# ShuangXieIrene/ssds.pytorch

Hardware: AMD Instinct MI355X
Metric: images/sec (fwd+decode+NMS) SSD-MobileNetV2@512 (higher is better)
Workload: dtype bf16

## Files before the change

ssds.pytorch_amd/csrc/ssdk_flow_common.h:

```cpp
#pragma once
#include "ssdk_common.h"

namespace ssdk {

typedef __bf16 fl_bf16x8 __attribute__((ext_vector_type(8)));
typedef _Float16 fl_f16x8 __attribute__((ext_vector_type(8)));
typedef float f32x4 __attribute__((ext_vector_type(4)));
typedef _Float16 fl_h2 __attribute__((ext_vector_type(2)));

struct FlowParams {
  const u16* x;
  u16* y;
  const u16* we;
  const float* se;
  const float* be;
  const u16* wd;
  const u16* bd;
  const u16* wp;
  const float* sp;
  const float* bp;
  int N, H, W, Cin, Chid, Cout, Ho, Wo, residual;
  int strips, segs, rs;
  int Himg, Wimg, Cimg, layout;
  unsigned long long seg_mask;
// ... 13 lines not shown
  if constexpr (DT == SSDK_BF16) {
    u32 b = __builtin_bit_cast(u32, v);
    if ((b & 0x7fffffffu) > 0x7f800000u) return (b >> 16) | 0x40u;
    return (b + 0x7fffu + ((b >> 16) & 1u)) >> 16;
  } else {
    _Float16 h = (_Float16)v;
    return (u32)__builtin_bit_cast(u16, h);
  }
}
typedef float fl_f32x2 __attribute__((ext_vector_type(2)));
typedef __bf16 fl_bf16x2 __attribute__((ext_vector_type(2)));
template <int DT> __device__ __forceinline__ u32 fl_pack2(float a, float b) {
  const fl_f32x2 v = {a, b};
  if constexpr (DT == SSDK_BF16) return __builtin_bit_cast(u32, __builtin_convertvector(v, fl_bf16x2));
  else return __builtin_bit_cast(u32, __builtin_convertvector(v, fl_h2));
}
template <int DT> __device__ __forceinline__ float fl_from16(u32 h) {
  if constexpr (DT == SSDK_BF16) return bf16_bits_to_f32(h);
  else return f16_bits_to_f32(h);
}
__device__ __forceinline__ u32 fl_from_left(u32 v) { return (u32)__builtin_amdgcn_update_dpp(0, (int)v, 0x111, 0xf, 0xf, true); }
__device__ __forceinline__ u32 fl_from_right(u32 v) { return (u32)__builtin_amdgcn_update_dpp(0, (int)v, 0x101, 0xf, 0xf, true); }

typedef float fl_f2 __attribute__((ext_vector_type(2)));
constexpr float kFlSixth = 1.0f / 6.0f;
__device__ __forceinline__ u32 fl_unit_pack(float a, float b, fl_f2 k) {
  const fl_f2 v = {a, b};
  fl_f2 r;
  asm("v_pk_mul_f32 %0, %1, %2 clamp" : "=v"(r) : "v"(v), "v"(k));
  return __builtin_bit_cast(u32, __builtin_amdgcn_cvt_pkrtz(r[0], r[1]));
}
__device__ __forceinline__ fl_h2 fl_fma_clamp01(fl_h2 a, fl_h2 b, fl_h2 c) {
  fl_h2 r;
  asm("v_pk_fma_f16 %0, %1, %2, %3 clamp" : "=v"(r) : "v"(a), "v"(b), "v"(c));
  return r;
}
__device__ __forceinline__ u32 fl_sixth_h2(u32 w) {
  return fl_to16<SSDK_F16>(fl_from16<SSDK_F16>(w & 0xffffu) * kFlSixth) | (fl_to16<SSDK_F16>(fl_from16<SSDK_F16>(w >> 16) * kFlSixth) << 16);
}

}
```

ssds.pytorch_amd/csrc/ssdk_mbflow.hip:

```cpp
#include <stdio.h>
#include <atomic>
#include <type_traits>

#include "ssdk_common.h"
#include "ssdk_flow_common.h"

namespace ssdk {

constexpr int kFlowThreads = 256;

template <int NCH, int NFO>
struct FlowLds {
  static constexpr int T = (NCH + 1) / 2;
  static constexpr int we = 0;
  static constexpr int sb = we + NCH * 1024;
  static constexpr int wd = sb + NCH * 4 * 32;
  static constexpr int bd = wd + NCH * 9 * 4 * 8;
  static constexpr int wp = (bd + NCH * 4 * 8 + 15) & ~15;
  static constexpr int spb = wp + NFO * T * 1024;
  static constexpr int bytes = spb + NFO * 4 * 32;
};

template <int DT, int S, int NCH, int NFO, int NS, bool STEM = false, bool YE = false, bool PAIR = false, bool XD = false>
__global__ __launch_bounds__(kFlowThreads, ((STEM && !YE) || PAIR) ? 3 : 2) void mbflow_kernel(const FlowParams p) {
  static_assert(!PAIR || (S == 1 && !STEM), "row pairs: stride-1 blocks");
  static_assert(!XD || (STEM && !YE), "dword image loads: the stem's interior instance");
  using L = FlowLds<NCH, NFO>;
  constexpr int T = L::T;
  extern __shared__ __attribute__((aligned(16))) unsigned char smem[];
  const u32 tid = threadIdx.x, lane = tid & 63u, wave = tid >> 6;
  const u32 fr = lane & 15u, fg = lane >> 4;
  const int Cin = p.Cin, Chid = p.Chid, Cout = p.Cout;

  for (u32 i = tid; i < (u32)(NCH * 64); i += kFlowThreads) {
    const u32 c = i >> 6, l = i & 63u, hc = c * 16 + (l & 15u), k0 = (l >> 4) * 8;
    u32x4 v = {0u, 0u, 0u, 0u};
    if constexpr (STEM) {
      if (hc < (u32)Chid) {
#pragma unroll
        for (u32 j = 0; j < 8; ++j) {
          u32 ci, ky, kx;
          bool kv;
          if constexpr (XD) {
            const u32 g = k0 >> 3;
            u32 t;
            if (j < 3u) {
              t = 2u * g;
              kx = j == 2u ? 0u : j + 1u;
// ... 72 lines not shown
    }
    *reinterpret_cast<f32x4*>(smem + L::spb + i * 32) = s;
    *reinterpret_cast<f32x4*>(smem + L::spb + i * 32 + 16) = b;
  }
  __syncthreads();

  const u32 item = blockIdx.x * (kFlowThreads / 64) + (u32)__builtin_amdgcn_readfirstlane((int)wave);
  const int groups = (p.strips + NS - 1) / NS;
  const int nseg = STEM ? __builtin_popcountll(p.seg_mask) : p.segs;
  const u32 per_img = (u32)(groups * nseg);
  if (item >= (u32)p.N * per_img) return;
  const int n = (int)(item / per_img), rem = (int)(item % per_img);
  int seg = rem / groups;
  const int grp = rem % groups;
  if constexpr (STEM) {
    unsigned long long m = p.seg_mask;
    for (int i = 0; i < seg; ++i) m &= m - 1;
    seg = __builtin_ctzll(m);
  }
  constexpr int OW = S == 1 ? 14 : 7;
  constexpr bool MERGE = S == 2 && NS == 2;
  constexpr int NA = MERGE ? 1 : NS;
  const int oy0 = seg * p.rs, oy1 = (oy0 + p.rs < p.Ho ? oy0 + p.rs : p.Ho) - 1;
  int ix[NS], oxl[NA];
  bool col_ok[NS], out_lane[NA];
#pragma unroll
  for (int s = 0; s < NS; ++s) {
    const int strip = grp * NS + s;
    const int ox0 = strip * OW;
    ix[s] = MERGE ? 2 * (grp * 15 + (int)fr) - s : ox0 * S - 1 + (int)fr;
    col_ok[s] = strip < p.strips && (unsigned)ix[s] < (unsigned)p.W;
    if constexpr (!MERGE) {
      oxl[s] = S == 1 ? ox0 + (int)fr - 1 : ox0 + ((int)fr - 1) / 2;
      out_lane[s] = strip < p.strips && (S == 1 ? (fr >= 1u && fr <= 14u) : ((fr & 1u) && fr <= 13u)) && oxl[s] < p.Wo;
    }
  }
  if constexpr (MERGE) {
    oxl[0] = grp * 15 + (int)fr;
    out_lane[0] = fr <= 14u && oxl[0] < p.Wo;
  }

  const u16* ximg = STEM ? p.x + (size_t)n * p.Cimg * p.Himg * p.Wimg : p.x + (size_t)n * p.H * p.W * Cin;
  const bool k_ok = fg * 8u < (u32)Cin;
  constexpr u32 kOOR = 0x40000000u;
  u32 xoff[STEM ? NS : 1][STEM ? 8 : 1], xoff0[(STEM && !YE) ? NS : 1][(STEM && !YE) ? 8 : 1], kyM[STEM ? 3 : 1];
  const int pstr = STEM ? (p.layout == 1 ? 1 : p.Cimg) : 0, cstr = STEM ? (p.layout == 1 ? p.Himg * p.Wimg : 1) : 0;
  if constexpr (STEM) {
    kyM[0] = kyM[1] = kyM[2] = 0u;
#pragma unroll
    for (int j = 0; j < 8; ++j) {
      const u32 k = fg * 8u + (u32)j, ci = k / 9u, ky = (k % 9u) / 3u, kx = k % 3u;
      const bool kv = k < 27u && ci < (u32)p.Cimg;
      const u32 vo = (u32)(2 * (int)fr * pstr + (int)ci * cstr + ((int)ky * p.Wimg + (int)kx) * pstr) * 2u;
      kyM[0] |= (kv && ky == 0u) ? (1u << j) : 0u;
      kyM[1] |= (kv && ky == 1u) ? (1u << j) : 0u;
      kyM[2] |= (kv && ky == 2u) ? (1u << j) : 0u;
#pragma unroll
      for (int s = 0; s < NS; ++s) {
        xoff[s][j] = (kv && col_ok[s] && (unsigned)(2 * ix[s] - 1 + (int)kx) < (unsigned)p.Wimg) ? vo : kOOR;
        if constexpr (!YE) xoff0[s][j] = ky == 0u ? kOOR : xoff[s][j];
      }
    }
  }
  u32 xd_off[XD ? NS : 1][3], xd_off0[XD ? NS : 1][2], xd_edge[2], xd_edge0[2];
  if constexpr (XD) {
    const u32 tA = 2u * fg, tB = 2u * fg + 1u;
    auto voff = [&](u32 t, int shift, int s_) -> u32 {
      const u32 ci = t / 3u, ky = t % 3u;
      const int px = ix[s_] - shift;
      const bool ok = ci < (u32)p.Cimg && grp * NS + s_ < p.strips && (unsigned)px < (unsigned)p.W;
      return ok ? (u32)((2 * (int)fr + (int)ci * p.Himg * p.Wimg + (int)ky * p.Wimg) * 2 + 4 * (1 - shift)) : kOOR;
    };
#pragma unroll
    for (int s = 0; s < NS; ++s) {
      xd_off[s][0] = voff(tA, 0, s);
      xd_off[s][1] = voff(tB, 0, s);
      xd_off[s][2] = fg == 0u ? voff(8u, 0, s) : (fg == 1u ? voff(8u, 1, s) : kOOR);
      xd_off0[s][0] = tA % 3u == 0u ? kOOR : xd_off[s][0];
      xd_off0[s][1] = tB % 3u == 0u ? kOOR : xd_off[s][1];
    }
    xd_edge[0] = fr == 0u ? voff(tA, 1, 0) : kOOR;
    xd_edge[1] = fr == 0u ? voff(tB, 1, 0) : kOOR;
    xd_edge0[0] = tA % 3u == 0u ? kOOR : xd_edge[0];
    xd_edge0[1] = tB % 3u == 0u ? kOOR : xd_edge[1];
  }
  const int xmargin = STEM ? (p.Wimg + 8) * pstr * 2 : 0;
  const __amdgpu_buffer_rsrc_t xrsrc = __builtin_amdgcn_make_buffer_rsrc(
      (void*)(reinterpret_cast<const unsigned char*>(ximg) - xmargin), 0, STEM ? p.Cimg * p.Himg * p.Wimg * 2 + xmargin : 0, 0x00020000);
  constexpr int XW = STEM ? 8 : 4;
  struct XRow {
    u32 w[XW];
  };
  auto load_x = [&](int iy, int s) -> XRow {
    XRow out;
#pragma unroll
    for (int q = 0; q < XW; ++q) out.w[q] = 0u;
    if constexpr (STEM) {
      const int strip = grp * NS + s;
      const int base = ((2 * iy - 1) * p.Wimg + (2 * (strip * 14 - 1) - 1)) * pstr;
      if constexpr (XD) {
        const bool row_in = (unsigned)iy < (unsigned)p.H, top = iy == 0;
        const int soff = row_in ? (base + 1) * 2 + xmargin - 4 : (int)kOOR;
        out.w[0] = (u32)__builtin_amdgcn_raw_buffer_load_b32(xrsrc, (int)(top ? xd_off0[s][0] : xd_off[s][0]), soff, 0);
        out.w[1] = (u32)__builtin_amdgcn_raw_buffer_load_b32(xrsrc, (int)(top ? xd_off0[s][1] : xd_off[s][1]), soff, 0);
        out.w[2] = (u32)__builtin_amdgcn_raw_buffer_load_b32(xrsrc, (int)xd_off[s][2], soff, 0);
        if (s == 0) {
          out.w[3] = (u32)__builtin_amdgcn_raw_buffer_load_b32(xrsrc, (int)(top ? xd_edge0[0] : xd_edge[0]), soff, 0);
          out.w[4] = (u32)__builtin_amdgcn_raw_buffer_load_b32(xrsrc, (int)(top ? xd_edge0[1] : xd_edge[1]), soff, 0);
        }
        return out;
      } else if constexpr (YE) {
        u32 rowmask = 0;
#pragma unroll
        for (int ky = 0; ky < 3; ++ky)
          rowmask |= ((unsigned)iy < (unsigned)p.H && (unsigned)(2 * iy - 1 + ky) < (unsigned)p.Himg) ? kyM[ky] : 0u;
#pragma unroll
        for (int j = 0; j < 8; ++j) {
          const u32 off = (((rowmask >> j) & 1u) && xoff[s][j] != kOOR) ? xoff[s][j] + (u32)(base * 2 + xmargin) : kOOR;
          out.w[j] = (u32)__builtin_amdgcn_raw_buffer_load_b16(xrsrc, (int)off, 0, 0);
        }
      } else {
        const bool row_in = (unsigned)iy < (unsigned)p.H, top = iy == 0;
        const int soff = row_in ? base * 2 + xmargin : (int)kOOR;
// ... 4 lines not shown
      return out;
    } else {
      if (k_ok && col_ok[s] && (unsigned)iy < (unsigned)p.H) {
        const u32x4 v = *reinterpret_cast<const u32x4*>(ximg + ((size_t)iy * p.W + ix[s]) * Cin + fg * 8);
        out.w[0] = v[0];
        out.w[1] = v[1];
        out.w[2] = v[2];
        out.w[3] = v[3];
      }
      return out;
    }
  };

  const bool dbgw = p.dbg != nullptr && blockIdx.x == gridDim.x / 2 && __builtin_amdgcn_readfirstlane((int)wave) == 0;
  int dbg_k = 0;
  fl_h2 accA[NA][NCH * 2], accB[NA][NCH * 2], accC[NA][NCH * 2];
  fl_h2 accD[PAIR ? NA : 1][PAIR ? NCH * 2 : 1];

  auto row = [&](const XRow (&xraw)[NS], int iy, auto FINc, auto MIDc, auto INIc, fl_h2 (&fin)[NA][NCH * 2],
                 fl_h2 (&mid)[NA][NCH * 2], fl_h2 (&ini)[NA][NCH * 2], int oy_fin) {
    constexpr bool FIN = decltype(FINc)::value, MID = decltype(MIDc)::value, INI = decltype(INIc)::value;
    if (dbgw && dbg_k < 250) {
      p.dbg[dbg_k++] = __builtin_readcyclecounter();
      if constexpr (STEM) asm volatile("s_waitcnt vmcnt(16)" ::: "memory");
      else asm volatile("s_waitcnt vmcnt(2)" ::: "memory");
      p.dbg[dbg_k++] = __builtin_readcyclecounter();
    }
    u32x4 xf[NS];
#pragma unroll
    for (int s = 0; s < NS; ++s) {
      if constexpr (XD) {
        int oa, ob;
        if (s == 0) {
          oa = (int)xraw[0].w[3];
          ob = (int)xraw[0].w[4];
        } else {
          oa = __builtin_amdgcn_update_dpp(0, (int)xraw[s - 1].w[0], 0x123, 0xf, 0xf, true);
          ob = __builtin_amdgcn_update_dpp(0, (int)xraw[s - 1].w[1], 0x123, 0xf, 0xf, true);
        }
        const u32 an = (u32)__builtin_amdgcn_update_dpp(oa, (int)xraw[s].w[0], 0x111, 0xf, 0xf, false);
        const u32 bn = (u32)__builtin_amdgcn_update_dpp(ob, (int)xraw[s].w[1], 0x111, 0xf, 0xf, false);
        xf[s][0] = xraw[s].w[0];
        xf[s][1] = __builtin_amdgcn_perm(bn, an, 0x07060302u);
        xf[s][2] = xraw[s].w[1];
        xf[s][3] = fg == 1u ? (xraw[s].w[2] & 0xffff0000u) : xraw[s].w[2];
      } else if constexpr (STEM) {
#pragma unroll
        for (int q = 0; q < 4; ++q) xf[s][q] = xraw[s].w[2 * q] | (xraw[s].w[2 * q + 1] << 16);
      } else {
#pragma unroll
        for (int q = 0; q < 4; ++q) xf[s][q] = xraw[s].w[q];
      }
    }
    fl_f2 hi[NS];
#pragma unroll
    for (int s = 0; s < NS; ++s) {
      const float k = (col_ok[s] && (unsigned)iy < (unsigned)p.H) ? kFlSixth : 0.f;
      hi[s] = fl_f2{k, k};
    }
    const bool store_row = FIN && oy_fin >= oy0 && oy_fin <= oy1;
    uint2 resv[NA][NFO];
    if (!STEM && !MERGE && FIN && store_row && p.residual) {
#pragma unroll
      for (int s = 0; s < NA; ++s)
#pragma unroll
        for (int f = 0; f < NFO; ++f) {
          const int co = f * 16 + (int)fg * 4;
          uint2 r = make_uint2(0u, 0u);
// ... 38 lines not shown
          fl_h2 s0 = init ? fl_as_h2(bdi.x) : a0, s1 = init ? fl_as_h2(bdi.y) : a1;
          s0 = __builtin_elementwise_fma(l0, fl_as_h2(w0.x), s0);
          s1 = __builtin_elementwise_fma(l1, fl_as_h2(w0.y), s1);
          s0 = __builtin_elementwise_fma(c0, fl_as_h2(w1.x), s0);
          s1 = __builtin_elementwise_fma(c1, fl_as_h2(w1.y), s1);
          if (ky == 2) {
            s0 = fl_fma_clamp01(r0, fl_as_h2(w2.x), s0);
            s1 = fl_fma_clamp01(r1, fl_as_h2(w2.y), s1);
          } else {
            s0 = __builtin_elementwise_fma(r0, fl_as_h2(w2.x), s0);
            s1 = __builtin_elementwise_fma(r1, fl_as_h2(w2.y), s1);
          }
          asm volatile("" : "+v"(s0), "+v"(s1));
          a0 = s0;
          a1 = s1;
        };
        if constexpr (INI) taps(0, ini[a][2 * c], ini[a][2 * c + 1], true);
        if constexpr (MID) taps(1, mid[a][2 * c], mid[a][2 * c + 1], false);
        if constexpr (FIN) taps(2, fin[a][2 * c], fin[a][2 * c + 1], false);
      };
      if constexpr (MERGE) {
        fold(fl_as_h2(ew[1][0]), fl_as_h2(ew[1][1]), fl_as_h2(ew[0][0]), fl_as_h2(ew[0][1]), fl_as_h2(fl_from_right(ew[1][0])),
             fl_as_h2(fl_from_right(ew[1][1])), 0);
      } else {
#pragma unroll
        for (int s = 0; s < NS; ++s)
          fold(fl_as_h2(fl_from_left(ew[s][0])), fl_as_h2(fl_from_left(ew[s][1])), fl_as_h2(ew[s][0]), fl_as_h2(ew[s][1]),
               fl_as_h2(fl_from_right(ew[s][0])), fl_as_h2(fl_from_right(ew[s][1])), s);
      }
#pragma unroll
      for (int s = 0; s < NS; ++s) e_cur[s] = e_nxt[s];
      __builtin_amdgcn_sched_barrier(0);
    }
    if (dbgw && dbg_k < 250) p.dbg[dbg_k++] = __builtin_readcyclecounter();
    if constexpr (FIN) {
      if (store_row) {
        asm volatile("" ::: "memory");
        f32x4 yacc[NA][NFO];
#pragma unroll
        for (int s = 0; s < NA; ++s)
#pragma unroll
          for (int f = 0; f < NFO; ++f) yacc[s][f] = f32x4{0.f, 0.f, 0.f, 0.f};
#pragma unroll
        for (int t = 0; t < T; ++t) {
          u32x4 db[NA];
#pragma unroll
// ... 196 lines not shown
          for (int o = 0; o < 2; ++o)
#pragma unroll
            for (int s = 0; s < NA; ++s) {
              if (!(st[o] && out_lane[s])) continue;
              u16* yrow = p.y + (((size_t)n * p.Ho + (iy - 1 + o)) * p.Wo + oxl[s]) * Cout;
              u32 h01 = fl_pack2<DT>(fmaf(yacc[o][s][f][0], spv[0], bpv[0]), fmaf(yacc[o][s][f][1], spv[1], bpv[1]));
              u32 h23 = fl_pack2<DT>(fmaf(yacc[o][s][f][2], spv[2], bpv[2]), fmaf(yacc[o][s][f][3], spv[3], bpv[3]));
              if (p.residual) {
                const u32 x01 = resv[o][s][f].x, x23 = resv[o][s][f].y;
                h01 = fl_pack2<DT>(fl_from16<DT>(h01 & 0xffffu) + fl_from16<DT>(x01 & 0xffffu), fl_from16<DT>(h01 >> 16) + fl_from16<DT>(x01 >> 16));
                h23 = fl_pack2<DT>(fl_from16<DT>(h23 & 0xffffu) + fl_from16<DT>(x23 & 0xffffu), fl_from16<DT>(h23 >> 16) + fl_from16<DT>(x23 >> 16));
              }
              *reinterpret_cast<uint2*>(yrow + co) = make_uint2(h01, h23);
            }
        }
      }
    }
    if (dbgw && dbg_k < 250) p.dbg[dbg_k++] = __builtin_readcyclecounter();
  };

  const auto Y = std::true_type{};
  const auto No = std::false_type{};
  auto load_row = [&](XRow (&dst)[NS], int iy) {
#pragma unroll
    for (int s = 0; s < NS; ++s) dst[s] = load_x(iy, s);
  };
  XRow xa[NS], xb[NS];
  {
    if constexpr (PAIR) {
      const int rend = oy1 + 1;
      XRow xc[NS], xd[NS];
      load_row(xa, oy0 - 1);
      load_row(xb, oy0);
      for (int r = oy0 - 1; r <= rend; r += 4) {
        load_row(xc, r + 2);
        load_row(xd, r + 3);
        row2(xa, xb, r, accA, accB, accC, accD);
        load_row(xa, r + 4);
        load_row(xb, r + 5);
        row2(xc, xd, r + 2, accC, accD, accA, accB);
      }
    } else if constexpr (S == 1) {
      const int rend = oy1 + 1;
      load_row(xa, oy0 - 1);
      for (int r = oy0 - 1; r <= rend; r += 6) {
        load_row(xb, r + 1);
// ... 8 lines not shown
        row(xa, r + 4, Y, Y, Y, accB, accC, accA, r + 3);
        load_row(xa, r + 6);
        row(xb, r + 5, Y, Y, Y, accC, accA, accB, r + 4);
      }
    } else {
      const int rend = 2 * oy1 + 1;
      load_row(xa, 2 * oy0 - 1);
      for (int r = 2 * oy0 - 1; r <= rend; r += 4) {
        load_row(xb, r + 1);
        row(xa, r, Y, No, Y, accA, accC, accB, (r - 1) / 2);
        load_row(xa, r + 2);
        row(xb, r + 1, No, Y, No, accC, accB, accC, 0);
        load_row(xb, r + 3);
        row(xa, r + 2, Y, No, Y, accB, accC, accA, (r + 1) / 2);
        load_row(xa, r + 4);
        row(xb, r + 3, No, Y, No, accC, accA, accC, 0);
      }
    }
  }
}

constexpr int kFlowNS = 2;

template <int DT, int S, int NCH, int NFO>
static void flow_launch(const FlowParams& p, unsigned grid, hipStream_t stream) {
  constexpr int lds = FlowLds<NCH, NFO>::bytes;
  if constexpr (S == 1 && NCH == 9) {
    if (p.layout == 101) {
      static const int pair = getenv("SSDK_FLOW_PAIR") ? atoi(getenv("SSDK_FLOW_PAIR")) : 1;
      if (pair) {
        (void)hipFuncSetAttribute(reinterpret_cast<const void*>(&mbflow_kernel<DT, S, NCH, NFO, 1, false, false, true>), hipFuncAttributeMaxDynamicSharedMemorySize, lds);
        hipLaunchKernelGGL((mbflow_kernel<DT, S, NCH, NFO, 1, false, false, true>), dim3(grid), dim3(kFlowThreads), lds, stream, p);
        return;
      }
      (void)hipFuncSetAttribute(reinterpret_cast<const void*>(&mbflow_kernel<DT, S, NCH, NFO, 1>), hipFuncAttributeMaxDynamicSharedMemorySize, lds);
      hipLaunchKernelGGL((mbflow_kernel<DT, S, NCH, NFO, 1>), dim3(grid), dim3(kFlowThreads), lds, stream, p);
      return;
    }
  }
  (void)hipFuncSetAttribute(reinterpret_cast<const void*>(&mbflow_kernel<DT, S, NCH, NFO, kFlowNS>), hipFuncAttributeMaxDynamicSharedMemorySize, lds);
  hipLaunchKernelGGL((mbflow_kernel<DT, S, NCH, NFO, kFlowNS>), dim3(grid), dim3(kFlowThreads), lds, stream, p);
}

template <int DT, int S>
static bool flow_dispatch(const FlowParams& p, int nch, int nfo, unsigned grid, hipStream_t stream) {
#define SSDK_FLOW(NCH_, NFO_)                                   \
  if (nch == NCH_ && nfo == NFO_) {                             \
    flow_launch<DT, S, NCH_, NFO_>(p, grid, stream);            \
    return true;                                                \
  }
  SSDK_FLOW(6, 2)
  SSDK_FLOW(9, 2)
  SSDK_FLOW(12, 2)
  SSDK_FLOW(12, 4)
#undef SSDK_FLOW
  return false;
}

int launch_mbflow(const ssdk_mbconv_desc* d, hipStream_t stream) {
// ... 45 lines not shown
    if (!dbg_dev) (void)hipMalloc(&dbg_dev, 256 * sizeof(unsigned long long));
    (void)hipMemsetAsync(dbg_dev, 0, 256 * sizeof(unsigned long long), stream);
    p.dbg = dbg_dev;
  }
  auto dbg_print = [&]() {
    if (!env_dbg) return;
    unsigned long long hh[256];
    (void)hipStreamSynchronize(stream);
    (void)hipMemcpy(hh, dbg_dev, sizeof(hh), hipMemcpyDeviceToHost);
    fprintf(stderr, "[mbflow dbg] Cin=%d Chid=%d Cout=%d s=%d stem=%d rs=%d: per row (wait x | chunks | project+store | to next row):", d->Cin,
            d->Chid, d->Cout, d->stride, (int)stem, p.rs);
    for (int i = 0; i + 4 < 250 && hh[i + 4]; i += 4)
      fprintf(stderr, " [%llu %llu %llu %llu]", hh[i + 1] - hh[i], hh[i + 2] - hh[i + 1], hh[i + 3] - hh[i + 2], hh[i + 4] - hh[i + 3]);
    fprintf(stderr, "\n");
  };
  const int ow = d->stride == 1 ? 14 : 7;
  p.strips = (p.Wo + ow - 1) / ow;
  if (d->stride == 2) p.strips = 2 * ((p.Wo + 14) / 15);
  constexpr int env_rs = 0;
  constexpr int env_ns1 = 1;
  const bool ns1 = ((env_ns1 & 1) && !stem && d->stride == 1 && nch == 9) || ((env_ns1 & 2) && stem);
  const int flow_ns = ns1 ? 1 : kFlowNS;
  if (ns1 && !stem) p.layout = 101;
  const int groups = (p.strips + flow_ns - 1) / flow_ns;
  int rs = 64;
  while (rs > 16 && (long)d->N * groups * ((p.Ho + rs - 1) / rs) < 4096) rs >>= 1;
  if ((long)d->N * groups * ((p.Ho + rs - 1) / rs) < 2048 && env_rs <= 0 && variant <= 0) return 1;
  if (variant > 0) {
    while (rs > 8 && (long)d->N * groups * ((p.Ho + rs - 1) / rs) < 2048) rs >>= 1;
  }
  if (env_rs > 0) rs = env_rs;
  if (rs > p.Ho) rs = p.Ho;
  p.rs = rs;
  p.segs = (p.Ho + rs - 1) / rs;
  const long items = (long)d->N * groups * p.segs;
  const unsigned grid = (unsigned)((items + 3) / 4);
  bool ok;
  if (stem) {
    if (p.segs > 64) return 1;
    unsigned long long edge = 0;
    for (int sgi = 0; sgi < p.segs; ++sgi) {
      const int o0 = sgi * p.rs, o1 = (o0 + p.rs < p.Ho ? o0 + p.rs : p.Ho) - 1;
      const int last_row = o1 + 1 < p.H - 1 ? o1 + 1 : p.H - 1;
      if (2 * last_row + 1 >= p.Himg) edge |= 1ull << sgi;
    }
    const unsigned long long all = p.segs == 64 ? ~0ull : ((1ull << p.segs) - 1ull);
    constexpr int lds = FlowLds<2, 1>::bytes;
    auto go = [&](auto DTc, auto YEc, unsigned long long mask) {
      constexpr int DTv = decltype(DTc)::value;
      constexpr bool YEv = decltype(YEc)::value;
      if (!mask) return;
      FlowParams q = p;
      q.seg_mask = mask;
      const long it = (long)d->N * groups * __builtin_popcountll(mask);
      const unsigned g = (unsigned)((it + 3) / 4);
      if (ns1) {
        (void)hipFuncSetAttribute(reinterpret_cast<const void*>(&mbflow_kernel<DTv, 1, 2, 1, 1, true, YEv>),
                                  hipFuncAttributeMaxDynamicSharedMemorySize, lds);
        hipLaunchKernelGGL((mbflow_kernel<DTv, 1, 2, 1, 1, true, YEv>), dim3(g), dim3(kFlowThreads), lds, stream, q);
        return;
      }
      if constexpr (!YEv) {
        static const int env_xd = getenv("SSDK_STEM_DWORD") ? atoi(getenv("SSDK_STEM_DWORD")) : 1;
        if (env_xd && q.layout == 1 && (q.Wimg & 1) == 0 && (reinterpret_cast<uintptr_t>(q.x) & 3u) == 0) {
          (void)hipFuncSetAttribute(reinterpret_cast<const void*>(&mbflow_kernel<DTv, 1, 2, 1, kFlowNS, true, false, false, true>),
                                    hipFuncAttributeMaxDynamicSharedMemorySize, lds);
          hipLaunchKernelGGL((mbflow_kernel<DTv, 1, 2, 1, kFlowNS, true, false, false, true>), dim3(g), dim3(kFlowThreads), lds, stream, q);
          return;
        }
      }
      (void)hipFuncSetAttribute(reinterpret_cast<const void*>(&mbflow_kernel<DTv, 1, 2, 1, kFlowNS, true, YEv>),
                                hipFuncAttributeMaxDynamicSharedMemorySize, lds);
      hipLaunchKernelGGL((mbflow_kernel<DTv, 1, 2, 1, kFlowNS, true, YEv>), dim3(g), dim3(kFlowThreads), lds, stream, q);
    };
    if (d->dtype == SSDK_BF16) {
      go(std::integral_constant<int, SSDK_BF16>{}, std::false_type{}, all & ~edge);
      go(std::integral_constant<int, SSDK_BF16>{}, std::true_type{}, edge);
    } else {
      go(std::integral_constant<int, SSDK_F16>{}, std::false_type{}, all & ~edge);
      go(std::integral_constant<int, SSDK_F16>{}, std::true_type{}, edge);
    }
    dbg_print();
    return 0;
  }
  if (d->dtype == SSDK_BF16) ok = d->stride == 1 ? flow_dispatch<SSDK_BF16, 1>(p, nch, nfo, grid, stream) : flow_dispatch<SSDK_BF16, 2>(p, nch, nfo, grid, stream);
  else ok = d->stride == 1 ? flow_dispatch<SSDK_F16, 1>(p, nch, nfo, grid, stream) : flow_dispatch<SSDK_F16, 2>(p, nch, nfo, grid, stream);
  if (ok) dbg_print();
// ... 5 lines not shown
```

ssds.pytorch_amd/csrc/ssdk_mbk.hip:

```cpp
#include "ssdk_common.h"
#include "ssdk_flow_common.h"
#include "ssdk_scan.h"

namespace ssdk {

struct MbkParams {
  const u16* x;
  u16* y;
  const unsigned char* img;
  int N, H, W, Ho, Wo, Cin, Chid, Cout, residual;
  int pairs, halves;
  unsigned items;
  unsigned long long* dbg;
  unsigned wave_mask, pair_mask;
};

template <int KS, int NW, int NCHW, int NFO>
struct MbkGeo {
  static constexpr int NP = (NCHW + 1) / 2;
  static constexpr int PAIR_KB = 2 * KS + NFO;
  static constexpr int MISC_KB = (NCHW * 384 + 1023) / 1024;
  static constexpr int m_be = 0, m_wd = NCHW * 64, m_bd = NCHW * (64 + 288);
  static constexpr int SPB_KB = 2;
  static_assert(NFO * 128 <= SPB_KB * 1024, "projection BN block");
// ... 22 lines not shown
  static constexpr int xch = spb + G::SPB_KB * 1024;
  static constexpr int bytes = xch + NW * XF * 1024;
};

__device__ __forceinline__ void mbk_mfma_guard() {
  __builtin_amdgcn_sched_barrier(0);
  asm volatile("s_nop 15\n\ts_nop 3" ::: "memory");
  __builtin_amdgcn_sched_barrier(0);
}
__device__ __forceinline__ void mbk_valu_guard() {
  __builtin_amdgcn_sched_barrier(0);
  asm volatile("s_nop 3" ::: "memory");
  __builtin_amdgcn_sched_barrier(0);
}
__device__ __forceinline__ u32 fl_from_left2(u32 cur, u32 prev) {
  const int old = __builtin_amdgcn_update_dpp(0, (int)prev, 0x121, 0xf, 0xf, true);
  return (u32)__builtin_amdgcn_update_dpp(old, (int)cur, 0x111, 0xf, 0xf, false);
}
__device__ __forceinline__ u32 fl_from_right2(u32 cur, u32 next) {
  const int old = __builtin_amdgcn_update_dpp(0, (int)next, 0x12f, 0xf, 0xf, true);
  return (u32)__builtin_amdgcn_update_dpp(old, (int)cur, 0x101, 0xf, 0xf, false);
}

template <int DT, int S, int NS, int KS, int NW, int NCHW, int NFO, bool DBG = false>
__global__ __launch_bounds__(64 * NW, 2) void mbk_kernel(const MbkParams p) {
  using L = MbkLds<S, NS, KS, NW, NCHW, NFO>;
  using G = MbkGeo<KS, NW, NCHW, NFO>;
  using I = MbkItem<S, NS>;
  constexpr int NR = I::NR, NXS = I::NXS, NE = NR * NXS;
  constexpr int XF = L::XF, FT = L::FT, NP = G::NP, PAIR_KB = G::PAIR_KB;
  constexpr int NO = 2 * NS;
  constexpr bool ODD = (NCHW & 1) != 0;
  constexpr int ROUNDS = FT / XF;
  extern __shared__ __attribute__((aligned(16))) unsigned char smem[];
  const u32 tid = threadIdx.x, lane = tid & 63u;
  const u32 fr = lane & 15u, fg = lane >> 4;
  const int wv = __builtin_amdgcn_readfirstlane((int)(tid >> 6));
  const int Cin = p.Cin, Cout = p.Cout, H = p.H, W = p.W, Ho = p.Ho, Wo = p.Wo;

  const u32 item = blockIdx.x;
  const int half = (int)(item % (u32)p.halves);
  const u32 rem = item / (u32)p.halves;
  const int n = (int)(rem / (u32)p.pairs), rp = (int)(rem % (u32)p.pairs);
  const int oy0 = 2 * rp;
  const int iy0 = S * oy0 - 1;
  const int co_base = half * 16 * NFO;
  const u16* ximg = p.x + (size_t)n * H * W * Cin;
  const bool stamp = p.dbg != nullptr && blockIdx.x == 0 && tid == 0;
  if (stamp) p.dbg[0] = __builtin_readcyclecounter();

  const u32x4* wimg = reinterpret_cast<const u32x4*>(p.img + ((size_t)(half * NW + wv) * NP) * ((size_t)PAIR_KB * 1024)) + lane;
  u32x4 wa[KS], wb[KS];
#pragma unroll
  for (int ks = 0; ks < KS; ++ks) {
    wa[ks] = wimg[(size_t)ks * 64];
    wb[ks] = wimg[(size_t)(KS + ks) * 64];
  }

  for (int e = wv; e < NE; e += NW) {
    const int r = e / NXS, xs = e % NXS;
    int iy = iy0 + r;
    iy = iy < 0 ? 0 : (iy > H - 1 ? H - 1 : iy);
    const int col = S == 1 ? 16 * xs + (int)fr : 2 * (16 * (xs >> 1) + (int)fr) + (xs & 1);
    const u16* src = ximg + ((size_t)iy * W + col) * Cin + fg * 8;
#pragma unroll
    for (int ks = 0; ks < KS; ++ks)
      __builtin_amdgcn_global_load_lds((glb_u8*)(src + ks * 32), (lds_u8*)(smem + L::xt + (e * KS + ks) * 1024), 16, 0, 0);
  }
  {
    const unsigned char* src = p.img + G::misc_off(p.halves) + (size_t)wv * (G::MISC_KB * 1024) + lane * 16;
#pragma unroll
    for (int k = 0; k < G::MISC_KB; ++k)
      __builtin_amdgcn_global_load_lds((glb_u8*)(src + k * 1024), (lds_u8*)(smem + L::misc + (wv * G::MISC_KB + k) * 1024), 16, 0, 0);
  }
  if (wv == 0) {
    const unsigned char* src = p.img + G::spb_off(p.halves) + (size_t)half * (G::SPB_KB * 1024) + lane * 16;
#pragma unroll
    for (int k = 0; k < G::SPB_KB; ++k)
      __builtin_amdgcn_global_load_lds((glb_u8*)(src + k * 1024), (lds_u8*)(smem + L::spb + k * 1024), 16, 0, 0);
  }
  asm volatile("s_waitcnt vmcnt(0)" ::: "memory");
  __syncthreads();
  if (stamp) p.dbg[1] = __builtin_readcyclecounter();

  fl_f2 hi[NR];
#pragma unroll
// ... 29 lines not shown
    for (int t = 0; t < 9; ++t) wt[t] = *reinterpret_cast<const uint2*>(mc + G::m_wd + ((c * 9 + t) * 4 + (int)fg) * 8);
    const uint2 bdi = *reinterpret_cast<const uint2*>(mc + G::m_bd + (c * 4 + (int)fg) * 8);
    mbk_mfma_guard();
    u32 ew[NR][NXS][2];
#pragma unroll
    for (int r = 0; r < NR; ++r)
#pragma unroll
      for (int xs = 0; xs < NXS; ++xs) {
        ew[r][xs][0] = fl_unit_pack(e[r * NXS + xs][0], e[r * NXS + xs][1], hi[r]);
        ew[r][xs][1] = fl_unit_pack(e[r * NXS + xs][2], e[r * NXS + xs][3], hi[r]);
      }
#pragma unroll
    for (int o = 0; o < 2; ++o)
#pragma unroll
      for (int j = 0; j < NS; ++j) {
        fl_h2 s[2] = {fl_as_h2(bdi.x), fl_as_h2(bdi.y)};
#pragma unroll
        for (int ky = 0; ky < 3; ++ky) {
          const int r = S * o + ky;
          const uint2 w0 = wt[ky * 3], w1 = wt[ky * 3 + 1], w2 = wt[ky * 3 + 2];
#pragma unroll
          for (int wd = 0; wd < 2; ++wd) {
            u32 tl, tc, tr;
            if constexpr (S == 1) {
              tc = ew[r][j][wd];
              tl = j == 0 ? fl_from_left(tc) : fl_from_left2(tc, ew[r][j > 0 ? j - 1 : 0][wd]);
              tr = j == NS - 1 ? fl_from_right(tc) : fl_from_right2(tc, ew[r][j < NS - 1 ? j + 1 : j][wd]);
            } else {
              const u32 odd = ew[r][2 * j + 1][wd];
              tc = ew[r][2 * j][wd];
              tl = j == 0 ? fl_from_left(odd) : fl_from_left2(odd, ew[r][j > 0 ? 2 * j - 1 : 1][wd]);
              tr = odd;
            }
            const u32 ww0 = wd ? w0.y : w0.x, ww1 = wd ? w1.y : w1.x, ww2 = wd ? w2.y : w2.x;
            s[wd] = __builtin_elementwise_fma(fl_as_h2(tl), fl_as_h2(ww0), s[wd]);
            s[wd] = __builtin_elementwise_fma(fl_as_h2(tc), fl_as_h2(ww1), s[wd]);
            if (ky == 2) s[wd] = fl_fma_clamp01(fl_as_h2(tr), fl_as_h2(ww2), s[wd]);
            else s[wd] = __builtin_elementwise_fma(fl_as_h2(tr), fl_as_h2(ww2), s[wd]);
          }
        }
        dout[o * NS + j][0] = fl_as_u32(s[0]);
        dout[o * NS + j][1] = fl_as_u32(s[1]);
      }
  };

  constexpr int FH = NFO / 2;
  for (int t = 0; t < NP; ++t) {
// ... 34 lines not shown
#pragma unroll
    for (int f = 0; f < NFO; ++f)
#pragma unroll
      for (int o = 0; o < NO; ++o)
        yacc[o][f] = fl_mfma<SSDK_F16>(f < FH ? wf0[f < FH ? f : 0] : wf1[f >= FH ? f - FH : 0], db[o], yacc[o][f]);
    __builtin_amdgcn_sched_barrier(0);
#pragma unroll
    for (int ks = 0; ks < KS; ++ks) {
      wa[ks] = na[ks];
      wb[ks] = nb[ks];
    }
  }
  if (stamp) p.dbg[2] = __builtin_readcyclecounter();

  unsigned char* xb = smem + L::xch;
  const unsigned char* spb = smem + L::spb;
  constexpr int GPW = (XF + NW - 1) / NW;
  uint2 resv[ROUNDS][GPW];
#pragma unroll
  for (int R = 0; R < ROUNDS; ++R)
#pragma unroll
    for (int gg = 0; gg < GPW; ++gg) {
      const int g = wv + gg * NW, q = R * XF + g, oj = q / NFO, f = q % NFO;
      const int oy = oy0 + oj / NS, ox = 16 * (oj % NS) + (int)fr, co = co_base + f * 16 + (int)fg * 4;
      resv[R][gg] = make_uint2(0u, 0u);
      if (S == 1 && p.residual && g < XF && oy < Ho && co < Cout)
        resv[R][gg] = *reinterpret_cast<const uint2*>(ximg + ((size_t)oy * W + ox) * Cin + co);
    }
#pragma unroll
  for (int R = 0; R < ROUNDS; ++R) {
#pragma unroll
    for (int g = 0; g < XF; ++g) {
      const int q = R * XF + g, oj = q / NFO, f = q % NFO;
      *reinterpret_cast<f32x4*>(xb + ((wv * XF + g) * 64 + (int)lane) * 16) = yacc[oj][f];
    }
    __syncthreads();
#pragma unroll
    for (int gg = 0; gg < GPW; ++gg) {
      const int g = wv + gg * NW;
      if (g < XF) {
        const int q = R * XF + g, oj = q / NFO, f = q % NFO;
        f32x4 y = *reinterpret_cast<const f32x4*>(xb + ((0 * XF + g) * 64 + (int)lane) * 16);
#pragma unroll
        for (int w2 = 1; w2 < NW; ++w2) {
          const f32x4 t2 = *reinterpret_cast<const f32x4*>(xb + ((w2 * XF + g) * 64 + (int)lane) * 16);
          y = y + t2;
        }
        const int oy = oy0 + oj / NS, ox = 16 * (oj % NS) + (int)fr;
        const int co = co_base + f * 16 + (int)fg * 4;
        if (oy < Ho && co < Cout) {
          const f32x4 spv = *reinterpret_cast<const f32x4*>(spb + (f * 4 + (int)fg) * 32);
          const f32x4 bpv = *reinterpret_cast<const f32x4*>(spb + (f * 4 + (int)fg) * 32 + 16);
          u32 h01 = fl_pack2<DT>(fmaf(y[0], spv[0], bpv[0]), fmaf(y[1], spv[1], bpv[1]));
          u32 h23 = fl_pack2<DT>(fmaf(y[2], spv[2], bpv[2]), fmaf(y[3], spv[3], bpv[3]));
          if (S == 1 && p.residual) {
            const uint2 xr = resv[R][gg];
            h01 = fl_pack2<DT>(fl_from16<DT>(h01 & 0xffffu) + fl_from16<DT>(xr.x & 0xffffu), fl_from16<DT>(h01 >> 16) + fl_from16<DT>(xr.x >> 16));
            h23 = fl_pack2<DT>(fl_from16<DT>(h23 & 0xffffu) + fl_from16<DT>(xr.y & 0xffffu), fl_from16<DT>(h23 >> 16) + fl_from16<DT>(xr.y >> 16));
          }
          u16* yrow = p.y + (((size_t)n * Ho + oy) * Wo + ox) * Cout;
          *reinterpret_cast<uint2*>(yrow + co) = make_uint2(h01, h23);
        }
      }
    }
    if (R + 1 < ROUNDS) __syncthreads();
  }
  if (stamp) p.dbg[3] = __builtin_readcyclecounter();
}

template <int DT, int S, int NS, int KS, int NW, int NCHW, int NFO, bool DBG = false>
static void mbk_launch(const MbkParams& p, hipStream_t stream) {
  constexpr int lds = MbkLds<S, NS, KS, NW, NCHW, NFO>::bytes;
  static_assert(lds <= 160 * 1024, "LDS");
  (void)hipFuncSetAttribute(reinterpret_cast<const void*>(&mbk_kernel<DT, S, NS, KS, NW, NCHW, NFO, DBG>),
                            hipFuncAttributeMaxDynamicSharedMemorySize, lds);
  hipLaunchKernelGGL((mbk_kernel<DT, S, NS, KS, NW, NCHW, NFO, DBG>), dim3(p.items), dim3(64 * NW), lds, stream, p);
}

constexpr int kMbkNW = 4;
struct MbkInst {
  int s, ns, ks, nchw, nfo;
};
static const MbkInst kMbkInst[] = {{1, 1, 5, 15, 10}, {2, 1, 3, 9, 10}, {1, 2, 2, 6, 4}, {1, 2, 2, 6, 6}, {1, 2, 3, 9, 6},
                                   {2, 2, 1, 3, 4}, {1, 4, 1, 3, 2}};

static int mbk_find(int stride, int Wo, int Cin, int Chid, int Cout, int nw, int* halves) {
  if (nw != kMbkNW || Cin % 32 || Chid % 16 || Cout % 16 || Wo % 16) return -1;
  const int ks = Cin / 32, nch = Chid / 16, nchw = (nch + nw - 1) / nw, ns = Wo / 16;
  for (int i = 0; i < (int)(sizeof(kMbkInst) / sizeof(kMbkInst[0])); ++i) {
    const MbkInst& k = kMbkInst[i];
    if (k.s == stride && k.ns == ns && k.ks == ks && k.nchw == nchw && Cout % (16 * k.nfo) == 0) {
      if (halves) *halves = Cout / (16 * k.nfo);
      return i;
    }
  }
  return -1;
// ... 97 lines not shown
```

Measured before the change: 64170.

## Interleave strip columns across lanes so depthwise neighbours come from registers

Adds an interleaved column mapping in which lane fr of strip q owns column NS*fr+q. Horizontal depthwise neighbours then mostly come from the sibling strip's register, with a single DPP shift instead of two-input DPP merges. It is enabled for the mbk kernel by default (env bit 1), and optionally for the flow kernel and stem (bit 2) with paired 64-bit image loads. This cuts cross-lane shuffles and halo columns at the cost of strided global access patterns, which may coalesce less well.

```diff
diff --git a/ssds.pytorch_amd/csrc/ssdk_flow_common.h b/ssds.pytorch_amd/csrc/ssdk_flow_common.h
--- a/ssds.pytorch_amd/csrc/ssdk_flow_common.h
+++ b/ssds.pytorch_amd/csrc/ssdk_flow_common.h
@@ -59,6 +59,22 @@
 __device__ __forceinline__ u32 fl_from_left(u32 v) { return (u32)__builtin_amdgcn_update_dpp(0, (int)v, 0x111, 0xf, 0xf, true); }
 __device__ __forceinline__ u32 fl_from_right(u32 v) { return (u32)__builtin_amdgcn_update_dpp(0, (int)v, 0x101, 0xf, 0xf, true); }
 
+inline int fl_interleave_env() {
+  static const int v = getenv("SSDK_FLOW_INTERLEAVE") ? atoi(getenv("SSDK_FLOW_INTERLEAVE")) : 1;
+  return v;
+}
+template <int NS> __device__ __forceinline__ int fl_il_col(int c0, int fr, int q) { return c0 + NS * fr + q; }
+template <int NS> __device__ __forceinline__ void fl_il_from_left(const u32 (&v)[NS], u32 (&l)[NS]) {
+  l[0] = fl_from_left(v[NS - 1]);
+#pragma unroll
+  for (int q = 1; q < NS; ++q) l[q] = v[q - 1];
+}
+template <int NS> __device__ __forceinline__ void fl_il_from_right(const u32 (&v)[NS], u32 (&r)[NS]) {
+#pragma unroll
+  for (int q = 0; q + 1 < NS; ++q) r[q] = v[q + 1];
+  r[NS - 1] = fl_from_right(v[0]);
+}
+
 typedef float fl_f2 __attribute__((ext_vector_type(2)));
 constexpr float kFlSixth = 1.0f / 6.0f;
 __device__ __forceinline__ u32 fl_unit_pack(float a, float b, fl_f2 k) {
diff --git a/ssds.pytorch_amd/csrc/ssdk_mbflow.hip b/ssds.pytorch_amd/csrc/ssdk_mbflow.hip
--- a/ssds.pytorch_amd/csrc/ssdk_mbflow.hip
+++ b/ssds.pytorch_amd/csrc/ssdk_mbflow.hip
@@ -21,9 +21,10 @@
   static constexpr int bytes = spb + NFO * 4 * 32;
 };
 
-template <int DT, int S, int NCH, int NFO, int NS, bool STEM = false, bool YE = false, bool PAIR = false, bool XD = false>
+template <int DT, int S, int NCH, int NFO, int NS, bool STEM = false, bool YE = false, bool PAIR = false, bool XD = false, bool IL = false>
 __global__ __launch_bounds__(kFlowThreads, ((STEM && !YE) || PAIR) ? 3 : 2) void mbflow_kernel(const FlowParams p) {
   static_assert(!PAIR || (S == 1 && !STEM), "row pairs: stride-1 blocks");
+  static_assert(!IL || (S == 1 && NS >= 2 && !PAIR), "interleaved strips: stride 1, several strips per wave");
   static_assert(!XD || (STEM && !YE), "dword image loads: the stem's interior instance");
   using L = FlowLds<NCH, NFO>;
   constexpr int T = L::T;
@@ -142,15 +143,24 @@
   constexpr bool MERGE = S == 2 && NS == 2;
   constexpr int NA = MERGE ? 1 : NS;
   const int oy0 = seg * p.rs, oy1 = (oy0 + p.rs < p.Ho ? oy0 + p.rs : p.Ho) - 1;
+  constexpr bool XP = XD && IL;
+  static_assert(!XP || NS == 2, "pair loads: two strips per wave");
+  constexpr int GW = XP ? 28 : 16 * NS - 2;
+  auto lcol = [&](int s) -> int { return IL ? NS * (int)fr + s : (int)fr; };
+  auto col0 = [&](int s) -> int { return IL ? grp * GW - (XP ? 2 : 1) : (grp * NS + s) * OW * S - 1; };
   int ix[NS], oxl[NA];
   bool col_ok[NS], out_lane[NA];
 #pragma unroll
   for (int s = 0; s < NS; ++s) {
     const int strip = grp * NS + s;
     const int ox0 = strip * OW;
-    ix[s] = MERGE ? 2 * (grp * 15 + (int)fr) - s : ox0 * S - 1 + (int)fr;
+    ix[s] = MERGE ? 2 * (grp * 15 + (int)fr) - s : (IL ? fl_il_col<NS>(col0(s), (int)fr, s) : ox0 * S - 1 + (int)fr);
     col_ok[s] = strip < p.strips && (unsigned)ix[s] < (unsigned)p.W;
-    if constexpr (!MERGE) {
+    if constexpr (IL) {
+      oxl[s] = ix[s];
+      const bool halo = XP ? (fr == 0u || fr == 15u) : ((s == 0 && fr == 0u) || (s == NS - 1 && fr == 15u));
+      out_lane[s] = strip < p.strips && !halo && oxl[s] < p.Wo;
+    } else if constexpr (!MERGE) {
       oxl[s] = S == 1 ? ox0 + (int)fr - 1 : ox0 + ((int)fr - 1) / 2;
       out_lane[s] = strip < p.strips && (S == 1 ? (fr >= 1u && fr <= 14u) : ((fr & 1u) && fr <= 13u)) && oxl[s] < p.Wo;
     }
@@ -171,12 +181,13 @@
     for (int j = 0; j < 8; ++j) {
       const u32 k = fg * 8u + (u32)j, ci = k / 9u, ky = (k % 9u) / 3u, kx = k % 3u;
       const bool kv = k < 27u && ci < (u32)p.Cimg;
-      const u32 vo = (u32)(2 * (int)fr * pstr + (int)ci * cstr + ((int)ky * p.Wimg + (int)kx) * pstr) * 2u;
+      const u32 vk = (u32)((int)ci * cstr + ((int)ky * p.Wimg + (int)kx) * pstr) * 2u;
       kyM[0] |= (kv && ky == 0u) ? (1u << j) : 0u;
       kyM[1] |= (kv && ky == 1u) ? (1u << j) : 0u;
       kyM[2] |= (kv && ky == 2u) ? (1u << j) : 0u;
 #pragma unroll
       for (int s = 0; s < NS; ++s) {
+        const u32 vo = vk + (u32)(2 * lcol(s) * pstr) * 2u;
         xoff[s][j] = (kv && col_ok[s] && (unsigned)(2 * ix[s] - 1 + (int)kx) < (unsigned)p.Wimg) ? vo : kOOR;
         if constexpr (!YE) xoff0[s][j] = ky == 0u ? kOOR : xoff[s][j];
       }
@@ -189,13 +200,13 @@
       const u32 ci = t / 3u, ky = t % 3u;
       const int px = ix[s_] - shift;
       const bool ok = ci < (u32)p.Cimg && grp * NS + s_ < p.strips && (unsigned)px < (unsigned)p.W;
-      return ok ? (u32)((2 * (int)fr + (int)ci * p.Himg * p.Wimg + (int)ky * p.Wimg) * 2 + 4 * (1 - shift)) : kOOR;
+      return ok ? (u32)((2 * lcol(s_) + (int)ci * p.Himg * p.Wimg + (int)ky * p.Wimg) * 2 + 4 * (1 - shift)) : kOOR;
     };
 #pragma unroll
     for (int s = 0; s < NS; ++s) {
       xd_off[s][0] = voff(tA, 0, s);
       xd_off[s][1] = voff(tB, 0, s);
-      xd_off[s][2] = fg == 0u ? voff(8u, 0, s) : (fg == 1u ? voff(8u, 1, s) : kOOR);
+      xd_off[s][2] = fg == 0u ? voff(8u, 0, s) : (fg == 1u ? voff(8u, XP ? 0 : 1, s) : kOOR);
       xd_off0[s][0] = tA % 3u == 0u ? kOOR : xd_off[s][0];
       xd_off0[s][1] = tB % 3u == 0u ? kOOR : xd_off[s][1];
     }
@@ -216,9 +227,10 @@
 #pragma unroll
     for (int q = 0; q < XW; ++q) out.w[q] = 0u;
     if constexpr (STEM) {
-      const int strip = grp * NS + s;
-      const int base = ((2 * iy - 1) * p.Wimg + (2 * (strip * 14 - 1) - 1)) * pstr;
-      if constexpr (XD) {
+      const int base = ((2 * iy - 1) * p.Wimg + (2 * col0(s) - 1)) * pstr;
+      if constexpr (XP) {
+        return out;
+      } else if constexpr (XD) {
         const bool row_in = (unsigned)iy < (unsigned)p.H, top = iy == 0;
         const int soff = row_in ? (base + 1) * 2 + xmargin - 4 : (int)kOOR;
         out.w[0] = (u32)__builtin_amdgcn_raw_buffer_load_b32(xrsrc, (int)(top ? xd_off0[s][0] : xd_off[s][0]), soff, 0);
@@ -269,7 +281,8 @@
     constexpr bool FIN = decltype(FINc)::value, MID = decltype(MIDc)::value, INI = decltype(INIc)::value;
     if (dbgw && dbg_k < 250) {
       p.dbg[dbg_k++] = __builtin_readcyclecounter();
-      if constexpr (STEM) asm volatile("s_waitcnt vmcnt(16)" ::: "memory");
+      if constexpr (XP) asm volatile("s_waitcnt vmcnt(3)" ::: "memory");
+      else if constexpr (STEM) asm volatile("s_waitcnt vmcnt(16)" ::: "memory");
       else asm volatile("s_waitcnt vmcnt(2)" ::: "memory");
       p.dbg[dbg_k++] = __builtin_readcyclecounter();
     }
@@ -277,20 +290,31 @@
 #pragma unroll
     for (int s = 0; s < NS; ++s) {
       if constexpr (XD) {
-        int oa, ob;
-        if (s == 0) {
-          oa = (int)xraw[0].w[3];
-          ob = (int)xraw[0].w[4];
+        u32 an, bn, cn = 0u;
+        if (XP && s > 0) {
+          an = xraw[s > 0 ? s - 1 : 0].w[0];
+          bn = xraw[s > 0 ? s - 1 : 0].w[1];
+          cn = xraw[s > 0 ? s - 1 : 0].w[2];
+        } else if constexpr (XP) {
+          an = fl_from_left(xraw[NS - 1].w[0]);
+          bn = fl_from_left(xraw[NS - 1].w[1]);
+          cn = fl_from_left(xraw[NS - 1].w[2]);
         } else {
-          oa = __builtin_amdgcn_update_dpp(0, (int)xraw[s - 1].w[0], 0x123, 0xf, 0xf, true);
-          ob = __builtin_amdgcn_update_dpp(0, (int)xraw[s - 1].w[1], 0x123, 0xf, 0xf, true);
-        }
-        const u32 an = (u32)__builtin_amdgcn_update_dpp(oa, (int)xraw[s].w[0], 0x111, 0xf, 0xf, false);
-        const u32 bn = (u32)__builtin_amdgcn_update_dpp(ob, (int)xraw[s].w[1], 0x111, 0xf, 0xf, false);
+          int oa, ob;
+          if (s == 0) {
+            oa = (int)xraw[0].w[3];
+            ob = (int)xraw[0].w[4];
+          } else {
+            oa = __builtin_amdgcn_update_dpp(0, (int)xraw[s > 0 ? s - 1 : 0].w[0], 0x123, 0xf, 0xf, true);
+            ob = __builtin_amdgcn_update_dpp(0, (int)xraw[s > 0 ? s - 1 : 0].w[1], 0x123, 0xf, 0xf, true);
+          }
+          an = (u32)__builtin_amdgcn_update_dpp(oa, (int)xraw[s].w[0], 0x111, 0xf, 0xf, false);
+          bn = (u32)__builtin_amdgcn_update_dpp(ob, (int)xraw[s].w[1], 0x111, 0xf, 0xf, false);
+        }
         xf[s][0] = xraw[s].w[0];
         xf[s][1] = __builtin_amdgcn_perm(bn, an, 0x07060302u);
         xf[s][2] = xraw[s].w[1];
-        xf[s][3] = fg == 1u ? (xraw[s].w[2] & 0xffff0000u) : xraw[s].w[2];
+        xf[s][3] = fg == 1u ? ((XP ? cn : xraw[s].w[2]) & 0xffff0000u) : xraw[s].w[2];
       } else if constexpr (STEM) {
 #pragma unroll
         for (int q = 0; q < 4; ++q) xf[s][q] = xraw[s].w[2 * q] | (xraw[s].w[2 * q + 1] << 16);
@@ -375,6 +399,20 @@
       if constexpr (MERGE) {
         fold(fl_as_h2(ew[1][0]), fl_as_h2(ew[1][1]), fl_as_h2(ew[0][0]), fl_as_h2(ew[0][1]), fl_as_h2(fl_from_right(ew[1][0])),
              fl_as_h2(fl_from_right(ew[1][1])), 0);
+      } else if constexpr (IL) {
+        u32 v0[NS], v1[NS], l0[NS], l1[NS], r0[NS], r1[NS];
+#pragma unroll
+        for (int s = 0; s < NS; ++s) {
+          v0[s] = ew[s][0];
+          v1[s] = ew[s][1];
+        }
+        fl_il_from_left<NS>(v0, l0);
+        fl_il_from_left<NS>(v1, l1);
+        fl_il_from_right<NS>(v0, r0);
+        fl_il_from_right<NS>(v1, r1);
+#pragma unroll
+        for (int s = 0; s < NS; ++s)
+          fold(fl_as_h2(l0[s]), fl_as_h2(l1[s]), fl_as_h2(v0[s]), fl_as_h2(v1[s]), fl_as_h2(r0[s]), fl_as_h2(r1[s]), s);
       } else {
 #pragma unroll
         for (int s = 0; s < NS; ++s)
@@ -617,6 +655,23 @@
   const auto Y = std::true_type{};
   const auto No = std::false_type{};
   auto load_row = [&](XRow (&dst)[NS], int iy) {
+    if constexpr (XP) {
+      const bool row_in = (unsigned)iy < (unsigned)p.H, top = iy == 0;
+      const int base = (2 * iy - 1) * p.Wimg + (2 * col0(0) - 1);
+      const int soff = row_in ? (base + 1) * 2 + xmargin - 4 : (int)kOOR;
+      const auto a = __builtin_amdgcn_raw_buffer_load_b64(xrsrc, (int)(top ? xd_off0[0][0] : xd_off[0][0]), soff, 0);
+      const auto b = __builtin_amdgcn_raw_buffer_load_b64(xrsrc, (int)(top ? xd_off0[0][1] : xd_off[0][1]), soff, 0);
+      const auto c = __builtin_amdgcn_raw_buffer_load_b64(xrsrc, (int)xd_off[0][2], soff, 0);
+#pragma unroll
+      for (int s = 0; s < 2; ++s) {
+#pragma unroll
+        for (int q = 0; q < XW; ++q) dst[s < NS ? s : 0].w[q] = 0u;
+        dst[s < NS ? s : 0].w[0] = (u32)a[s];
+        dst[s < NS ? s : 0].w[1] = (u32)b[s];
+        dst[s < NS ? s : 0].w[2] = (u32)c[s];
+      }
+      return;
+    }
 #pragma unroll
     for (int s = 0; s < NS; ++s) dst[s] = load_x(iy, s);
   };
@@ -671,6 +726,8 @@
 
 constexpr int kFlowNS = 2;
 
+static bool flow_interleaved(int stride, int ns) { return stride == 1 && ns >= 2 && (fl_interleave_env() & 2) != 0; }
+
 template <int DT, int S, int NCH, int NFO>
 static void flow_launch(const FlowParams& p, unsigned grid, hipStream_t stream) {
   constexpr int lds = FlowLds<NCH, NFO>::bytes;
@@ -684,6 +741,13 @@
       }
       (void)hipFuncSetAttribute(reinterpret_cast<const void*>(&mbflow_kernel<DT, S, NCH, NFO, 1>), hipFuncAttributeMaxDynamicSharedMemorySize, lds);
       hipLaunchKernelGGL((mbflow_kernel<DT, S, NCH, NFO, 1>), dim3(grid), dim3(kFlowThreads), lds, stream, p);
+      return;
+    }
+  }
+  if constexpr (S == 1) {
+    if (flow_interleaved(S, kFlowNS)) {
+      (void)hipFuncSetAttribute(reinterpret_cast<const void*>(&mbflow_kernel<DT, S, NCH, NFO, kFlowNS, false, false, false, false, true>), hipFuncAttributeMaxDynamicSharedMemorySize, lds);
+      hipLaunchKernelGGL((mbflow_kernel<DT, S, NCH, NFO, kFlowNS, false, false, false, false, true>), dim3(grid), dim3(kFlowThreads), lds, stream, p);
       return;
     }
   }
@@ -775,6 +839,8 @@
   const bool ns1 = ((env_ns1 & 1) && !stem && d->stride == 1 && nch == 9) || ((env_ns1 & 2) && stem);
   const int flow_ns = ns1 ? 1 : kFlowNS;
   if (ns1 && !stem) p.layout = 101;
+  const bool il = !stem && flow_interleaved(d->stride, flow_ns);
+  if (il) p.strips = flow_ns * ((p.Wo + 16 * flow_ns - 3) / (16 * flow_ns - 2));
   const int groups = (p.strips + flow_ns - 1) / flow_ns;
   int rs = 64;
   while (rs > 16 && (long)d->N * groups * ((p.Ho + rs - 1) / rs) < 4096) rs >>= 1;
@@ -816,6 +882,13 @@
       if constexpr (!YEv) {
         static const int env_xd = getenv("SSDK_STEM_DWORD") ? atoi(getenv("SSDK_STEM_DWORD")) : 1;
         if (env_xd && q.layout == 1 && (q.Wimg & 1) == 0 && (reinterpret_cast<uintptr_t>(q.x) & 3u) == 0) {
+          if (flow_interleaved(1, kFlowNS) && (q.W & 1) == 0) {
+            q.strips = kFlowNS * groups;
+            (void)hipFuncSetAttribute(reinterpret_cast<const void*>(&mbflow_kernel<DTv, 1, 2, 1, kFlowNS, true, false, false, true, true>),
+                                      hipFuncAttributeMaxDynamicSharedMemorySize, lds);
+            hipLaunchKernelGGL((mbflow_kernel<DTv, 1, 2, 1, kFlowNS, true, false, false, true, true>), dim3(g), dim3(kFlowThreads), lds, stream, q);
+            return;
+          }
           (void)hipFuncSetAttribute(reinterpret_cast<const void*>(&mbflow_kernel<DTv, 1, 2, 1, kFlowNS, true, false, false, true>),
                                     hipFuncAttributeMaxDynamicSharedMemorySize, lds);
           hipLaunchKernelGGL((mbflow_kernel<DTv, 1, 2, 1, kFlowNS, true, false, false, true>), dim3(g), dim3(kFlowThreads), lds, stream, q);
diff --git a/ssds.pytorch_amd/csrc/ssdk_mbk.hip b/ssds.pytorch_amd/csrc/ssdk_mbk.hip
--- a/ssds.pytorch_amd/csrc/ssdk_mbk.hip
+++ b/ssds.pytorch_amd/csrc/ssdk_mbk.hip
@@ -68,8 +68,9 @@
   return (u32)__builtin_amdgcn_update_dpp(old, (int)cur, 0x101, 0xf, 0xf, false);
 }
 
-template <int DT, int S, int NS, int KS, int NW, int NCHW, int NFO, bool DBG = false>
+template <int DT, int S, int NS, int KS, int NW, int NCHW, int NFO, bool DBG = false, bool IL = false>
 __global__ __launch_bounds__(64 * NW, 2) void mbk_kernel(const MbkParams p) {
+  static_assert(!IL || (S == 1 && NS >= 2), "interleaved strips: stride 1, several strips per row");
   using L = MbkLds<S, NS, KS, NW, NCHW, NFO>;
   using G = MbkGeo<KS, NW, NCHW, NFO>;
   using I = MbkItem<S, NS>;
@@ -107,7 +108,7 @@
     const int r = e / NXS, xs = e % NXS;
     int iy = iy0 + r;
     iy = iy < 0 ? 0 : (iy > H - 1 ? H - 1 : iy);
-    const int col = S == 1 ? 16 * xs + (int)fr : 2 * (16 * (xs >> 1) + (int)fr) + (xs & 1);
+    const int col = S == 1 ? (IL ? fl_il_col<NS>(0, (int)fr, xs) : 16 * xs + (int)fr) : 2 * (16 * (xs >> 1) + (int)fr) + (xs & 1);
     const u16* src = ximg + ((size_t)iy * W + col) * Cin + fg * 8;
 #pragma unroll
     for (int ks = 0; ks < KS; ++ks)
@@ -183,7 +184,11 @@
 #pragma unroll
           for (int wd = 0; wd < 2; ++wd) {
             u32 tl, tc, tr;
-            if constexpr (S == 1) {
+            if constexpr (IL) {
+              tc = ew[r][j][wd];
+              tl = j == 0 ? fl_from_left(ew[r][NS - 1][wd]) : ew[r][j > 0 ? j - 1 : 0][wd];
+              tr = j == NS - 1 ? fl_from_right(ew[r][0][wd]) : ew[r][j < NS - 1 ? j + 1 : j][wd];
+            } else if constexpr (S == 1) {
               tc = ew[r][j][wd];
               tl = j == 0 ? fl_from_left(tc) : fl_from_left2(tc, ew[r][j > 0 ? j - 1 : 0][wd]);
               tr = j == NS - 1 ? fl_from_right(tc) : fl_from_right2(tc, ew[r][j < NS - 1 ? j + 1 : j][wd]);
@@ -264,7 +269,7 @@
 #pragma unroll
     for (int gg = 0; gg < GPW; ++gg) {
       const int g = wv + gg * NW, q = R * XF + g, oj = q / NFO, f = q % NFO;
-      const int oy = oy0 + oj / NS, ox = 16 * (oj % NS) + (int)fr, co = co_base + f * 16 + (int)fg * 4;
+      const int oy = oy0 + oj / NS, ox = IL ? fl_il_col<NS>(0, (int)fr, oj % NS) : 16 * (oj % NS) + (int)fr, co = co_base + f * 16 + (int)fg * 4;
       resv[R][gg] = make_uint2(0u, 0u);
       if (S == 1 && p.residual && g < XF && oy < Ho && co < Cout)
         resv[R][gg] = *reinterpret_cast<const uint2*>(ximg + ((size_t)oy * W + ox) * Cin + co);
@@ -288,7 +293,7 @@
           const f32x4 t2 = *reinterpret_cast<const f32x4*>(xb + ((w2 * XF + g) * 64 + (int)lane) * 16);
           y = y + t2;
         }
-        const int oy = oy0 + oj / NS, ox = 16 * (oj % NS) + (int)fr;
+        const int oy = oy0 + oj / NS, ox = IL ? fl_il_col<NS>(0, (int)fr, oj % NS) : 16 * (oj % NS) + (int)fr;
         const int co = co_base + f * 16 + (int)fg * 4;
         if (oy < Ho && co < Cout) {
           const f32x4 spv = *reinterpret_cast<const f32x4*>(spb + (f * 4 + (int)fg) * 32);
@@ -314,6 +319,14 @@
 static void mbk_launch(const MbkParams& p, hipStream_t stream) {
   constexpr int lds = MbkLds<S, NS, KS, NW, NCHW, NFO>::bytes;
   static_assert(lds <= 160 * 1024, "LDS");
+  if constexpr (S == 1 && NS >= 2 && !DBG) {
+    if (fl_interleave_env() & 1) {
+      (void)hipFuncSetAttribute(reinterpret_cast<const void*>(&mbk_kernel<DT, S, NS, KS, NW, NCHW, NFO, DBG, true>),
+                                hipFuncAttributeMaxDynamicSharedMemorySize, lds);
+      hipLaunchKernelGGL((mbk_kernel<DT, S, NS, KS, NW, NCHW, NFO, DBG, true>), dim3(p.items), dim3(64 * NW), lds, stream, p);
+      return;
+    }
+  }
   (void)hipFuncSetAttribute(reinterpret_cast<const void*>(&mbk_kernel<DT, S, NS, KS, NW, NCHW, NFO, DBG>),
                             hipFuncAttributeMaxDynamicSharedMemorySize, lds);
   hipLaunchKernelGGL((mbk_kernel<DT, S, NS, KS, NW, NCHW, NFO, DBG>), dim3(p.items), dim3(64 * NW), lds, stream, p);
```

Result: no change. 64810 (median of 4 runs) (+1.0%).
